# YuxiaWu/RAG4DyG

Measured on AMD Instinct MI355X. Metric: query-seqs/sec encode+top-k over full pool, higher is better.
Workload: dtype f32 (f16x2 operands: two fp16 terms, three products, f32 accumulate)

## Files before the change

### include/r4d.h

```cpp
#ifndef R4D_H
#define R4D_H

#include <stddef.h>
#include <stdint.h>

#ifdef __cplusplus
extern "C" {
#endif

#define R4D_OK 0
#define R4D_ERR_INVALID (-1)
#define R4D_ERR_HIP (-2)
#define R4D_ERR_WORKSPACE (-3)

#define R4D_ABI_VERSION 6

int r4d_abi_version(void);
int r4d_build_flags(void);
const char* r4d_last_error(void);

typedef struct r4d_gpt2_config {
    int32_t n_layer;
    int32_t n_head;
    int32_t n_embd;
// ... 13 lines not shown
    const float* c_fc_wT;     const float* mlp_proj_wT;
    const uint16_t* c_attn_w3;  const uint16_t* attn_proj_w3;
    const uint16_t* c_fc_w3;    const uint16_t* mlp_proj_w3;
    const uint16_t* c_attn_w3t; const uint16_t* attn_proj_w3t;
    const uint16_t* c_fc_w3t;   const uint16_t* mlp_proj_w3t;
    const float* c_attn_wTg;    const float* c_attn_lnc;
    const float* c_fc_wTg;      const float* c_fc_lnc;
    const uint16_t* c_attn_h2;  const uint16_t* attn_proj_h2;
    const uint16_t* c_fc_h2;    const uint16_t* mlp_proj_h2;
} r4d_gpt2_layer;

typedef struct r4d_gpt2_weights {
    const float* wte;
    const float* wpe;
    const float* ln_f_w;
    const float* ln_f_b;
    const r4d_gpt2_layer* layers;
    const float* lm_head;
} r4d_gpt2_weights;


size_t r4d_gpt2_workspace_bytes(const r4d_gpt2_config* cfg, int32_t B, int32_t T);

int r4d_gpt2_encode_f32(const r4d_gpt2_config* cfg, const r4d_gpt2_weights* w,
                        const int64_t* ids_d, const float* inputs_embeds_d, int32_t B, int32_t T,
                        float* out_hidden_d, float* out_meanpool_d, float* out_layers_d, float* out_qkv_d,
                        void* workspace_d, size_t workspace_bytes, void* stream);

size_t r4d_gpt2_groups_workspace_bytes(const r4d_gpt2_config* cfg, int32_t n_groups, const int32_t* Bs,
                                       const int32_t* Ts);
int r4d_gpt2_encode_groups_f32(const r4d_gpt2_config* cfg, const r4d_gpt2_weights* w, int32_t n_groups,
                               const int64_t* const* ids_d, const int32_t* Bs, const int32_t* Ts,
                               float* out_meanpool_d, void* workspace_d, size_t workspace_bytes, void* stream);

int r4d_gpt2_encode_groups_ex_f32(const r4d_gpt2_config* cfg, const r4d_gpt2_weights* w, int32_t n_groups,
                                  const int64_t* const* ids_d, const float* const* embeds_d, const int32_t* Bs,
                                  const int32_t* Ts, float* out_hidden_d, float* out_meanpool_d, float* out_qkv_d,
                                  void* workspace_d, size_t workspace_bytes, void* stream);

size_t r4d_gpt2_decode_workspace_bytes(const r4d_gpt2_config* cfg, int32_t B);
int r4d_gpt2_decode_step_f32(const r4d_gpt2_config* cfg, const r4d_gpt2_weights* w, const int64_t* ids_d,
                             const float* inputs_embeds_d, const int32_t* pos_d, float* kv_cache_d, int32_t B,
                             int32_t t_cap, float* out_hidden_d, void* workspace_d, size_t workspace_bytes,
                             void* stream);

typedef struct r4d_greedy_state {
    float* last_d;
    float* logits_d;
    int64_t* next_d;
    int32_t* lens_d;
    int32_t* pos_d;
    int32_t* active_d;
    int32_t* gen_len_d;
    int32_t* out_tokens_d;
    const int32_t* params_d;
    int32_t out_cap;
} r4d_greedy_state;
typedef struct r4d_decode_graph r4d_decode_graph;

size_t r4d_gpt2_greedy_workspace_bytes(const r4d_gpt2_config* cfg, int32_t B);
int r4d_gpt2_greedy_step_f32(const r4d_gpt2_config* cfg, const r4d_gpt2_weights* w, const r4d_greedy_state* st,
                             float* kv_cache_d, int32_t B, int32_t t_cap, void* workspace_d, size_t workspace_bytes,
                             void* stream);
int r4d_gpt2_greedy_graph_create(const r4d_gpt2_config* cfg, const r4d_gpt2_weights* w, const r4d_greedy_state* st,
                                 float* kv_cache_d, int32_t B, int32_t t_cap, void* workspace_d, size_t workspace_bytes,
                                 r4d_decode_graph** out_graph);
// ... 211 lines not shown
```

### rag4dyg_amd/_lib.py

```python
import ctypes
import os
from ctypes import POINTER, Structure, c_char_p, c_double, c_float, c_int32, c_int64, c_size_t, c_uint32, c_uint64, c_void_p

PKG = os.path.dirname(os.path.abspath(__file__))
LIB_PATH = os.environ.get("R4D_LIB_PATH") or os.path.join(PKG, "librag4dyg_hip.so")

R4D_ABI_VERSION = 6
HEAD_GRAD_UNTIED, HEAD_GRAD_TIED, HEAD_GRAD_NONE = 0, 1, 2


class R4DError(RuntimeError):
    pass


class GPT2ConfigC(Structure):
    _fields_ = [("n_layer", c_int32), ("n_head", c_int32), ("n_embd", c_int32), ("vocab", c_int32),
                ("n_positions", c_int32), ("ln_eps", c_float)]


class GPT2LayerC(Structure):
    _fields_ = [(n, c_void_p) for n in ("ln_1_w", "ln_1_b", "c_attn_w", "c_attn_b", "attn_proj_w", "attn_proj_b",
                                         "ln_2_w", "ln_2_b", "c_fc_w", "c_fc_b", "mlp_proj_w", "mlp_proj_b",
                                         "c_attn_wT", "attn_proj_wT", "c_fc_wT", "mlp_proj_wT",
                                         "c_attn_w3", "attn_proj_w3", "c_fc_w3", "mlp_proj_w3",
                                         "c_attn_w3t", "attn_proj_w3t", "c_fc_w3t", "mlp_proj_w3t",
                                         "c_attn_wTg", "c_attn_lnc", "c_fc_wTg", "c_fc_lnc",
                                         "c_attn_h2", "attn_proj_h2", "c_fc_h2", "mlp_proj_h2")]


class GreedyStateC(Structure):
    _fields_ = [(n, c_void_p) for n in ("last_d", "logits_d", "next_d", "lens_d", "pos_d", "active_d", "gen_len_d",
                                         "out_tokens_d", "params_d")] + [("out_cap", c_int32)]


class GPT2LayerGradsC(Structure):
    _fields_ = [(n, c_void_p) for n in ("ln_1_w", "ln_1_b", "c_attn_w", "c_attn_b", "attn_proj_w", "attn_proj_b",
                                         "ln_2_w", "ln_2_b", "c_fc_w", "c_fc_b", "mlp_proj_w", "mlp_proj_b")]


class TrainDropoutC(Structure):
    _fields_ = [("embd_p", c_float), ("attn_p", c_float), ("resid_p", c_float), ("seed", c_uint64), ("step", c_uint64)]


class GPT2GradsC(Structure):
    _fields_ = [("wte", c_void_p), ("wpe", c_void_p), ("ln_f_w", c_void_p), ("ln_f_b", c_void_p),
                ("layers", POINTER(GPT2LayerGradsC))]


class LMHeadC(Structure):
    _fields_ = [("wte_pad", c_void_p), ("ldV", c_int32), ("w3", c_void_p), ("w3t", c_void_p), ("h2", c_void_p)]


class GPT2WeightsC(Structure):
    _fields_ = [("wte", c_void_p), ("wpe", c_void_p), ("ln_f_w", c_void_p), ("ln_f_b", c_void_p),
                ("layers", POINTER(GPT2LayerC)), ("lm_head", c_void_p)]


_P = c_void_p
PROTOTYPES = {
    "r4d_abi_version": (c_int32, []),
    "r4d_build_flags": (c_int32, []),
    "r4d_last_error": (c_char_p, []),
    "r4d_gpt2_workspace_bytes": (c_size_t, [POINTER(GPT2ConfigC), c_int32, c_int32]),
    "r4d_gpt2_encode_f32": (c_int32, [POINTER(GPT2ConfigC), POINTER(GPT2WeightsC), _P, _P, c_int32, c_int32,
                                      _P, _P, _P, _P, _P, c_size_t, _P]),
    "r4d_gpt2_groups_workspace_bytes": (c_size_t, [POINTER(GPT2ConfigC), c_int32, POINTER(c_int32), POINTER(c_int32)]),
    "r4d_gpt2_encode_groups_f32": (c_int32, [POINTER(GPT2ConfigC), POINTER(GPT2WeightsC), c_int32, POINTER(_P),
                                             POINTER(c_int32), POINTER(c_int32), _P, _P, c_size_t, _P]),
    "r4d_gpt2_encode_groups_ex_f32": (c_int32, [POINTER(GPT2ConfigC), POINTER(GPT2WeightsC), c_int32, POINTER(_P), POINTER(_P),
                                                POINTER(c_int32), POINTER(c_int32), _P, _P, _P, _P, c_size_t, _P]),
    "r4d_set_attention_fused": (c_int32, [c_int32]),
    "r4d_set_attention_h2": (c_int32, [c_int32]),
    "r4d_set_attention_kblk": (c_int32, [c_int32]),
    "r4d_set_layer0_pad_rows": (c_int32, [c_int32]),
    "r4d_gpt2_layer0_pad_rows_offset": (c_size_t, [POINTER(GPT2ConfigC), c_int32, POINTER(c_int32), POINTER(c_int32)]),
    "r4d_pack_kblk_words": (c_int32, [_P, c_int64, c_int32, c_int32, _P, _P]),
    "r4d_attention_h2_kblk_f32": (c_int32, [_P, _P, c_int32, c_int32, c_int32, c_int32, _P, _P]),
    "r4d_set_range_flag": (c_int32, [_P]),
    "r4d_set_gemm_h2p": (c_int32, [c_int32]),
    "r4d_layernorm_lines_f32": (c_int32, [_P, _P, _P, c_int32, c_int32, c_float, _P, _P]),
    "r4d_split2_lines_f16": (c_int32, [_P, c_int64, c_int32, _P, _P]),
    "r4d_conv1d_h2p_f32": (c_int32, [_P, _P, _P, _P, c_int32, c_int32, c_int32, c_int32, c_int32, _P, _P]),
    "r4d_pack_h2_words_f32": (c_int32, [_P, c_int64, _P, _P]),
    "r4d_attention_h2_f32": (c_int32, [_P, c_int32, c_int32, c_int32, c_int32, _P, _P]),
    "r4d_gpt2_decode_workspace_bytes": (c_size_t, [POINTER(GPT2ConfigC), c_int32]),
    "r4d_gpt2_decode_step_f32": (c_int32, [POINTER(GPT2ConfigC), POINTER(GPT2WeightsC), _P, _P, _P, _P, c_int32, c_int32,
                                           _P, _P, c_size_t, _P]),
    "r4d_gpt2_greedy_workspace_bytes": (c_size_t, [POINTER(GPT2ConfigC), c_int32]),
    "r4d_gpt2_greedy_step_f32": (c_int32, [POINTER(GPT2ConfigC), POINTER(GPT2WeightsC), POINTER(GreedyStateC), _P, c_int32,
                                           c_int32, _P, c_size_t, _P]),
    "r4d_gpt2_greedy_graph_create": (c_int32, [POINTER(GPT2ConfigC), POINTER(GPT2WeightsC), POINTER(GreedyStateC), _P,
                                               c_int32, c_int32, _P, c_size_t, POINTER(_P)]),
    "r4d_decode_graph_launch": (c_int32, [_P, c_int32, _P]),
    "r4d_decode_graph_destroy": (None, [_P]),
    "r4d_lm_logits_f32": (c_int32, [_P, _P, c_int32, c_int32, c_int32, _P, _P]),
    "r4d_layernorm_f32": (c_int32, [_P, _P, _P, c_int32, c_int32, c_float, _P, _P]),
    "r4d_conv1d_f32": (c_int32, [_P, _P, _P, _P, _P, c_int32, c_int32, c_int32, c_int32, _P, _P]),
    "r4d_split3_planes_bf16": (c_int32, [_P, c_int32, c_int32, c_int32, _P, _P]),
    "r4d_conv1d_s3_f32": (c_int32, [_P, _P, _P, _P, c_int32, c_int32, c_int32, c_int32, _P, _P]),
    "r4d_split2_planes_f16": (c_int32, [_P, c_int32, c_int32, c_int32, _P, _P]),
    "r4d_conv1d_h2_f32": (c_int32, [_P, _P, _P, _P, c_int32, c_int32, c_int32, c_int32, _P, _P]),
    "r4d_fold_layernorm_f32": (c_int32, [_P, _P, _P, c_int32, c_int32, _P, _P, _P]),
    "r4d_set_gemm_split3": (c_int32, [c_int32]),
# ... 115 lines not shown
```

### rag4dyg_amd/csrc/common.h

```cpp
#pragma once
#include <hip/hip_runtime.h>
#include <stdint.h>
#include <stdio.h>
#include <stdarg.h>
#include "../../include/r4d.h"
#include "conv1d_route.h"

namespace r4d {

void set_error(const char* fmt, ...);
int dbgflag_kc(); int dbgflag_att(); int dbgflag_sk(); int dbgflag_jac(); int dbgflag_scan(); int dbgflag_s3(); int dbgflag_h2();

#define R4D_REQUIRE(cond, ...)                     \
    do {                                           \
        if (!(cond)) {                             \
            r4d::set_error(__VA_ARGS__);           \
            return R4D_ERR_INVALID;                \
        }                                          \
    } while (0)

#define R4D_HIP(call)                                                                  \
    do {                                                                               \
        hipError_t e_ = (call);                                                        \
        if (e_ != hipSuccess) {                                                        \
// ... 22 lines not shown
void prof_begin_impl(int cls, double work, hipStream_t s);
void prof_end_impl(hipStream_t s);
struct ProfScope {
    hipStream_t s; bool on;
    ProfScope(int cls, double work, hipStream_t st) : s(st), on(g_prof_on) { if (on) prof_begin_impl(cls, work, s); }
    ~ProfScope() { if (on) prof_end_impl(s); }
};

#define R4D_BRANCH_LIST(X)                                                                                              \
    X(KC_128x128x16, "gemm_kc:128x128x16") X(KC_128x64x16, "gemm_kc:128x64x16") X(KC_64x64x32, "gemm_kc:64x64x32")       \
    X(KC_128x128x32, "tuning:gemm_kc:128x128x32") X(KC_ROWSPLIT, "gemm_kc:row-split (two launches)")                      \
    X(S3_128x256, "gemm_s3:128x256x32") X(S3_PERSISTENT, "gemm_s3:128x256x32 persistent (pipeline across tiles)") X(S3_128x128, "gemm_s3:128x128x32") X(S3_F32B, "gemm_s3:both operands split on the fly (scoring GEMM)") X(S3_TN, "gemm_s3tn:128x256x32 (weight gradients, transposing LDS reads)")      \
    X(H2_128x256, "gemm_h2:128x256x32 (f16x2)") X(H2_128x128, "gemm_h2:128x128x32 (f16x2)") X(H2P_128x256, "gemm_h2p:128x256x32 (f16x2, A as lines, LDS-DMA)") X(H2P_128x128, "gemm_h2p:128x128x32 (f16x2, A as lines, LDS-DMA)") X(H2P_ROWMAP, "gemm_h2p:row-block map (layer 0 c_attn without the repeated pad-row blocks)") \
    X(F32_128x128, "gemm_f32:128x128") X(F32_128x64, "gemm_f32:128x64") X(F32_64x64, "gemm_f32:64x64")                   \
    X(F32_NT, "gemm_f32:B as [N,K]") X(F32_NN, "gemm_f32:B as [K,N]") X(TN_SPLITK, "gemm_tn:split-K") X(TN_SINGLE, "gemm_tn:one slice") \
    X(SK16_NG2, "skinny16:ng2") X(SK16_NG3, "skinny16:ng3") X(SK16_NG2_LN, "skinny16:ng2+layernorm") X(SK16_LN_FOLDED, "skinny16:LayerNorm pre-folded into the weight") X(SK16_NG3_LN, "skinny16:ng3+layernorm") \
    X(SK16_SPLITK, "skinny16:split-K last-arriver") X(SK8_NG2, "skinny8:ng2") X(SK8_NG3, "skinny8:ng3")                    \
    X(SK8_LN, "tuning:skinny8:+layernorm") X(SK8_SPLITK, "skinny8:split-K + epilogue launch") X(SK_PLAIN, "skinny:plain + epilogue launch") \
    X(ATT_KS32, "attention:key-split hd32") X(ATT_KS64, "attention:key-split hd64") X(ATT_CS96, "attention:column-split hd96") \
    X(ATT_CS128, "attention:column-split hd128") X(ATT_CS256, "attention:column-split hd256") X(ATT_H2_KS32, "attention:f16x2 key-split hd32") X(ATT_H2_KS64, "attention:f16x2 key-split hd64") X(ATT_H2_KS96, "attention:f16x2 key-split hd96") X(ATT_H2_128, "attention:f16x2 hd128") X(ATT_H2_256, "attention:f16x2 hd256") X(ATT_H2_KS32_KBLK, "attention:f16x2 key-split hd32, key-blocked K") X(ATT_H2_KS64_KBLK, "attention:f16x2 key-split hd64, key-blocked K") X(ATT_H2_KS96_KBLK, "attention:f16x2 key-split hd96, key-blocked K") X(ATT_H2_128_KBLK, "attention:f16x2 hd128, key-blocked K") X(ATT_H2_256_KBLK, "attention:f16x2 hd256, key-blocked K")                              \
    X(ATT_KS_FORCED, "tuning:attention:key-split at hd96/128/256") X(ATT_3LAUNCH, "attention:three-launch GEMM form")      \
    X(SCAN_1_1, "scan:d32") X(SCAN_2_1, "scan:d64") X(SCAN_4_1, "scan:d128") X(SCAN_4_2, "scan:d256") X(SCAN_4_3, "scan:d384") \
    X(SCAN_8_2, "scan:d512") X(SCAN_4_4, "tuning:scan:d512 4-way") X(SCAN_8_3, "scan:d768") X(SCAN_8_4, "scan:d1024")       \
    X(SCAN_SHORT, "scan:short shard (even rows, two tiles in flight)") X(SCAN_DMA, "scan:short shard, LDS-DMA staged") X(SCAN_RING, "scan:long shard, LDS-DMA ring") X(SCAN_GEMM, "scan:tiled GEMM (Q > 64 or other d)") X(SCAN_TILED, "scan:128x256 tiles in the scan kernels' arithmetic (Q >= 64)") X(SCAN_BF16X3, "scan:bf16x3 operands") X(SCAN_F32, "scan:exact-f32 operands")  \
    X(TOPK_ONE_WG, "topk:one workgroup per row") X(TOPK_TICKET, "topk:cross-workgroup ticket merge")                      \
    X(TOPK_MULTI, "topk:second launch over candidates") X(TOPK_F64, "topk:f64 rows")                                      \
    X(EMBED_LN4, "embed+layernorm:16-byte lanes") X(EMBED_GENERIC, "embed+layernorm:generic") X(LN4_2, "layernorm:ln4<2>") X(LN4_4, "layernorm:ln4<4>") X(LN4_8, "layernorm:ln4<8>") X(LN_GENERIC, "layernorm:generic") \
    X(LNF_8, "lnf_meanpool:<8>") X(LNF_16, "lnf_meanpool:<16>") X(LNF_32, "lnf_meanpool:<32>")                             \
    X(DEC_ATT_32, "decode_attention:<32>") X(DEC_ATT_64, "decode_attention:<64>")                                         \
    X(JAC_LDS, "jaccard:LDS table") X(JAC_MERGE, "jaccard:merge walk (vocab too large for LDS)")                          \
    X(JAC_PREP_DENSE_LDS, "jaccard_prep:dense tokens, LDS histogram") X(JAC_PREP_DENSE_GLOBAL, "jaccard_prep:dense tokens, global histogram") X(JAC_PREP_ORDER, "jaccard_prep:rows longest first") \
    X(ARGSORT_ONE, "argsort:one chunk") X(ARGSORT_MULTI, "argsort:chunk sort + rank scatter")                              \
    X(B1_128x256, "tuning:encode_bf16:128x256x32") X(B1_128x128, "tuning:encode_bf16:128x128x32")                           \
    X(TB_FWD, "tuning:train_bf16:fwd") X(TB_DGRAD, "tuning:train_bf16:dgrad") X(TB_WGRAD, "tuning:train_bf16:wgrad") X(TB_WGRAD_FALLBACK, "tuning:train_bf16:wgrad_fallback")
enum DispatchBranch {
#define X(id, name) BR_##id,
    R4D_BRANCH_LIST(X)
#undef X
    BR_COUNT
};
extern unsigned long long g_branch_hits[BR_COUNT];
#define R4D_BRANCH(id) (++r4d::g_branch_hits[r4d::BR_##id])

extern unsigned* g_range_flag;

static inline size_t align_up(size_t x, size_t a) { return (x + a - 1) / a * a; }

enum GemmCausal { CAUSAL_NONE = 0, CAUSAL_QK = 1, CAUSAL_PV = 2 };

struct GemmArgs {
    const float* A; const float* B; float* C;
    const float* bias;
    const float* resid;
    int M, N, K;
    int lda, ldb, ldc, ldr;
    int b_trans;
    int b_rows;
    int a_cols;
    int nbatch, nb1;
    long long sA0, sA1, sB0, sB1, sC0, sC1;
    int epilogue; float scale_div;
    int causal;
};
static inline GemmArgs gemm_args(const float* A, const float* B, int b_trans, const float* bias, const float* resid, int M, int K, int N,
                                 int epilogue, float* C) {
    GemmArgs g{};
    g.A = A; g.B = B; g.C = C; g.bias = bias; g.resid = resid;
// ... 184 lines not shown
```

### rag4dyg_amd/csrc/encoder.hip

```cpp
#include <math.h>
#include <stdlib.h>
#include <string.h>
#include <vector>
#include "common.h"

namespace r4d {

static thread_local char g_err[512] = "";
void set_error(const char* fmt, ...) {
    va_list ap;
    va_start(ap, fmt);
    vsnprintf(g_err, sizeof(g_err), fmt, ap);
    va_end(ap);
}

int g_gemm_split3 = 1;
int g_encode_bf16 = 0;

int conv1d(const Conv1DW& W, const float* x, const float* resid, int M, int epilogue, float* y, hipStream_t s, const Conv1DOpts& opts) {
    const int K = W.in, N = W.out;
    const GemmRoute route = conv1d_route(W, M, epilogue, opts.skinny_scratch != nullptr, opts.bf16);
    switch (route) {
        case ROUTE_B1:
            if (opts.bf16 == BF16_TRAIN) R4D_BRANCH(TB_FWD);
            return launch_gemm_b1(s3_args(x, W.w3, W.b, resid, M, K, N, epilogue, y), s);
        case ROUTE_SKINNY:
            return launch_gemm_skinny(x, W.wT, W.b, resid, M, K, N, epilogue, y, opts.skinny_scratch, s, nullptr, nullptr, 0.f,
                                      opts.counters_zeroed);
        case ROUTE_H2: return launch_gemm_h2(s3_args(x, W.h2, W.b, resid, M, K, N, epilogue, y), s);
        case ROUTE_S3: return launch_gemm_s3(s3_args(x, W.w3, W.b, resid, M, K, N, epilogue, y), s);
        default: break;
    }
    R4D_REQUIRE(epilogue != EPI_H2WORDS, "conv1d: the h2-word epilogue exists in the f16x2 GEMM only");
    const bool kcopy = route == ROUTE_F32_KCOPY;
    return launch_gemm_f32(gemm_args(x, kcopy ? W.wT : W.w, kcopy, W.b, resid, M, K, N, epilogue, y), s);
// ... 65 lines not shown
    size_t pad_rows_off;
    size_t bytes;
};
static Workspace carve(void* base, size_t M, size_t score_floats, size_t pool_floats, int d, const PadRowsPlan* pr = nullptr) {
    size_t off = 0;
    auto take = [&](size_t nfloat) {
        float* p = base ? (float*)((char*)base + off) : nullptr;
        off += align_up(nfloat * sizeof(float), 256);
        return p;
    };
    const size_t Mx = pr ? pr->rows() : M;
    Workspace w;
    w.x = take(Mx * d); w.ln = take(Mx * d); w.qkv = take(Mx * 3 * d); w.att = take(M * d); w.fc = take(M * 4 * d);
    w.scores = take(score_floats);
    w.pool = take(pool_floats);
    w.kblk = reinterpret_cast<unsigned*>(take(kblk_words(Mx, d)));
    w.pad_rows_off = off;
    w.pad_rows = pr ? reinterpret_cast<int*>(take(pr->words())) : nullptr;
    w.bytes = off;
    return w;
}
static int g_layer0_pad_rows = -1;
static int layer0_pad_rows_on() {
    if (g_layer0_pad_rows < 0) { const char* e = getenv("R4D_LAYER0_PAD_ROWS"); g_layer0_pad_rows = e ? atoi(e) != 0 : 1; }
    return g_layer0_pad_rows;
}
static PadRowsPlan groups_pad_rows_plan(const r4d_gpt2_config* cfg, size_t M, int n_groups, const int32_t* Ts) {
    int Tmax = 1;
    for (int g = 0; g < n_groups; ++g) Tmax = Ts[g] > Tmax ? Ts[g] : Tmax;
    return pad_rows_plan(M, Tmax, cfg->vocab > 0 ? cfg->vocab : 1);
}
static size_t score_floats(int B, int H, int T) { return (size_t)B * H * T * tpad(T); }

static int check_cfg(const r4d_gpt2_config* c) {
    R4D_REQUIRE(c != nullptr, "gpt2: null config");
    R4D_REQUIRE(c->n_layer >= 1 && c->n_head >= 1 && c->n_embd >= 64, "gpt2: bad config L=%d H=%d d=%d", c->n_layer,
                c->n_head, c->n_embd);
    R4D_REQUIRE(c->n_embd % 64 == 0 && c->n_embd <= 2048, "gpt2: n_embd=%d must be a multiple of 64, <= 2048", c->n_embd);
    R4D_REQUIRE(c->n_embd % c->n_head == 0 && (c->n_embd / c->n_head) % 16 == 0,
                "gpt2: head_dim=%d/%d must be a multiple of 16", c->n_embd, c->n_head);
    return R4D_OK;
}

}

using namespace r4d;

extern "C" {

int r4d_abi_version(void) { return R4D_ABI_VERSION; }
int r4d_build_flags(void) {
    return dbgflag_kc() | (dbgflag_att() << 1) | (dbgflag_sk() << 2) | (dbgflag_jac() << 3) | (dbgflag_scan() << 4) | (dbgflag_s3() << 5) | (dbgflag_h2() << 6) | (dbgflag_att_h2() << 7);
}
int r4d_fold_layernorm_f32(const float* wT_d, const float* ln_w_d, const float* ln_b_d, int32_t N, int32_t K, float* wTg_d,
                           float* lnc_d, void* stream) {
    return launch_fold_layernorm(wT_d, ln_w_d, ln_b_d, N, K, wTg_d, lnc_d, (hipStream_t)stream);
}

int r4d_set_gemm_split3(int32_t mode) { g_gemm_split3 = mode == 2 ? 2 : (mode != 0); return R4D_OK; }
int r4d_get_gemm_split3(void) { return g_gemm_split3; }
int r4d_set_encode_bf16(int32_t on) {
    const int prev = g_encode_bf16;
    g_encode_bf16 = on != 0;
    return prev;
}
int r4d_get_encode_bf16(void) { return g_encode_bf16; }
int r4d_set_range_flag(uint32_t* flag_d) { g_range_flag = flag_d; return R4D_OK; }
int r4d_set_attention_kblk(int32_t on) {
    const int prev = g_attention_kblk < 0 ? 1 : g_attention_kblk;
    g_attention_kblk = on != 0;
    return prev;
}
int r4d_set_attention_h2(int32_t on) {
    const int prev = g_attention_h2;
    g_attention_h2 = on != 0;
    return prev;
}

int r4d_set_attention_fused(int32_t mode) {
    g_attention_variant = (mode == 2) ? 1 : 0;
    g_attention_fused = mode < 0 ? -1 : (mode != 0);
    return R4D_OK;
}
const char* r4d_last_error(void) { return g_err; }

size_t r4d_gpt2_workspace_bytes(const r4d_gpt2_config* cfg, int32_t B, int32_t T) {
    if (!cfg || B <= 0 || T <= 0) return 0;
    const PadRowsPlan pr = groups_pad_rows_plan(cfg, (size_t)B * T, 1, &T);
    return carve(nullptr, (size_t)B * T, score_floats(B, cfg->n_head, T), lnf_meanpool_scratch_floats(B, T, cfg->n_embd),
                 cfg->n_embd, &pr).bytes;
}

size_t r4d_gpt2_groups_workspace_bytes(const r4d_gpt2_config* cfg, int32_t n_groups, const int32_t* Bs,
                                       const int32_t* Ts) {
    if (!cfg || n_groups <= 0 || !Bs || !Ts) return 0;
    size_t M = 0, sc = 0, pl = 0;
    for (int g = 0; g < n_groups; ++g) {
        if (Bs[g] <= 0 || Ts[g] <= 0) return 0;
        M += (size_t)Bs[g] * Ts[g];
        const size_t f = score_floats(Bs[g], cfg->n_head, Ts[g]);
        if (f > sc) sc = f;
        pl += lnf_meanpool_scratch_floats(Bs[g], Ts[g], cfg->n_embd);
    }
    const PadRowsPlan pr = groups_pad_rows_plan(cfg, M, n_groups, Ts);
    return carve(nullptr, M, sc, pl, cfg->n_embd, &pr).bytes;
}

size_t r4d_gpt2_layer0_pad_rows_offset(const r4d_gpt2_config* cfg, int32_t n_groups, const int32_t* Bs, const int32_t* Ts) {
    if (!cfg || n_groups <= 0 || !Bs || !Ts) return 0;
    size_t M = 0, sc = 0, pl = 0;
    for (int g = 0; g < n_groups; ++g) {
        if (Bs[g] <= 0 || Ts[g] <= 0) return 0;
        M += (size_t)Bs[g] * Ts[g];
        const size_t f = score_floats(Bs[g], cfg->n_head, Ts[g]);
        if (f > sc) sc = f;
        pl += lnf_meanpool_scratch_floats(Bs[g], Ts[g], cfg->n_embd);
    }
    const PadRowsPlan pr = groups_pad_rows_plan(cfg, M, n_groups, Ts);
    return carve(nullptr, M, sc, pl, cfg->n_embd, &pr).pad_rows_off;
}

int r4d_set_layer0_pad_rows(int32_t on) {
    const int prev = layer0_pad_rows_on();
    g_layer0_pad_rows = on != 0;
    return prev;
}

}

namespace r4d {

static int encode_impl(const r4d_gpt2_config* cfg, const r4d_gpt2_weights* w, const Group* groups, int n_groups,
                       float* out_hidden_d, float* out_meanpool_d, float* out_layers_d, float* out_qkv_d,
                       void* workspace_d, size_t workspace_bytes, hipStream_t s) {
    int rc = check_cfg(cfg);
    if (rc) return rc;
    R4D_REQUIRE(w && w->wte && w->wpe && w->ln_f_w && w->ln_f_b && w->layers, "gpt2: null weights");
    R4D_REQUIRE(out_hidden_d || out_meanpool_d, "gpt2: no output requested");
    const int d = cfg->n_embd, H = cfg->n_head;
    size_t Mtot = 0, sc = 0, pl = 0;
    int Tmax = 1;
    bool all_ids = true;
    for (int g = 0; g < n_groups; ++g) {
        const Group& G = groups[g];
        Tmax = G.T > Tmax ? G.T : Tmax;
        all_ids = all_ids && G.ids != nullptr;
        R4D_REQUIRE((G.ids != nullptr) != (G.emb != nullptr),
                    "gpt2: specify exactly one of input_ids and inputs_embeds");
        R4D_REQUIRE(G.B >= 1 && G.T >= 1, "gpt2: empty batch B=%d T=%d", G.B, G.T);
        R4D_REQUIRE(G.T <= cfg->n_positions && G.T <= 1024, "gpt2: T=%d exceeds n_positions=%d", G.T, cfg->n_positions);
        Mtot += (size_t)G.B * G.T;
        const size_t f = score_floats(G.B, H, G.T);
        if (f > sc) sc = f;
// ... 104 lines not shown
        }
        if (!fused_done) {
            for (int g = 0; g < n_groups; ++g) {
                const Group& G = groups[g];
                if ((rc = attention(qkv + G.row0 * 3 * d, G.B, G.T, H, d, ws.att + G.row0 * d, ws.scores, s))) return rc;
            }
        }
        if (att_lines) rc = conv1d_lines(Wo, reinterpret_cast<const unsigned short*>(ws.att), ws.x, M, EPI_RESIDUAL, ws.x, false, s);
        else rc = conv1d(Wo, ws.att, ws.x, M, EPI_RESIDUAL, ws.x, s, enc);
        if (rc) return rc;
        if (lines) {
            if ((rc = launch_layernorm_lines(ws.x, L.ln_2_w, L.ln_2_b, M, d, cfg->ln_eps, ln_lines, s))) return rc;
            if ((rc = conv1d_lines(Wfc, ln_lines, nullptr, M, EPI_GELU, fc_lines, true, s))) return rc;
            if ((rc = conv1d_lines(Wp, fc_lines, ws.x, M, EPI_RESIDUAL, ws.x, false, s))) return rc;
            continue;
        }
        if ((rc = launch_layernorm(ws.x, L.ln_2_w, L.ln_2_b, M, d, cfg->ln_eps, ws.ln, s))) return rc;
        if ((rc = conv1d(Wfc, ws.ln, nullptr, M, EPI_GELU, ws.fc, s, enc))) return rc;
        if ((rc = conv1d(Wp, ws.fc, ws.x, M, EPI_RESIDUAL, ws.x, s, enc))) return rc;
    }
    size_t part0 = 0;
    for (int g0 = 0; g0 < n_groups; g0 += ATT_MAXG) {
        const RowGroups R = row_groups(groups, g0, n_groups);
        const Group& G = groups[g0];
        rc = launch_lnf_meanpool_groups(R, ws.x + G.row0 * d, w->ln_f_w, w->ln_f_b, d, cfg->ln_eps,
                                        out_hidden_d ? out_hidden_d + G.row0 * d : nullptr,
                                        out_meanpool_d ? out_meanpool_d + G.seq0 * d : nullptr, ws.pool + part0, s);
        if (rc) return rc;
        for (int j = 0; j < R.n; ++j) part0 += lnf_meanpool_scratch_floats(R.B[j], R.T[j], d);
    }
    return R4D_OK;
}

}

extern "C" {

int r4d_gpt2_encode_f32(const r4d_gpt2_config* cfg, const r4d_gpt2_weights* w, const int64_t* ids_d,
                        const float* inputs_embeds_d, int32_t B, int32_t T, float* out_hidden_d,
                        float* out_meanpool_d, float* out_layers_d, float* out_qkv_d, void* workspace_d,
                        size_t workspace_bytes, void* stream) {
    Group G = {ids_d, inputs_embeds_d, B, T, 0, 0};
    return encode_impl(cfg, w, &G, 1, out_hidden_d, out_meanpool_d, out_layers_d, out_qkv_d, workspace_d,
                       workspace_bytes, (hipStream_t)stream);
}

int r4d_gpt2_encode_groups_f32(const r4d_gpt2_config* cfg, const r4d_gpt2_weights* w, int32_t n_groups,
                               const int64_t* const* ids_d, const int32_t* Bs, const int32_t* Ts,
                               float* out_meanpool_d, void* workspace_d, size_t workspace_bytes, void* stream) {
    R4D_REQUIRE(n_groups >= 1 && n_groups <= 4096 && ids_d && Bs && Ts, "gpt2 groups: bad arguments");
    R4D_REQUIRE(out_meanpool_d, "gpt2 groups: out_meanpool_d is null");
    std::vector<Group> gs((size_t)n_groups);
    size_t row0 = 0, seq0 = 0;
    for (int g = 0; g < n_groups; ++g) {
        gs[g] = Group{ids_d[g], nullptr, Bs[g], Ts[g], row0, seq0};
        if (Bs[g] > 0 && Ts[g] > 0) { row0 += (size_t)Bs[g] * Ts[g]; seq0 += (size_t)Bs[g]; }
    }
    return encode_impl(cfg, w, gs.data(), n_groups, nullptr, out_meanpool_d, nullptr, nullptr, workspace_d,
                       workspace_bytes, (hipStream_t)stream);
}

int r4d_gpt2_encode_groups_ex_f32(const r4d_gpt2_config* cfg, const r4d_gpt2_weights* w, int32_t n_groups,
                                  const int64_t* const* ids_d, const float* const* embeds_d, const int32_t* Bs,
                                  const int32_t* Ts, float* out_hidden_d, float* out_meanpool_d, float* out_qkv_d,
                                  void* workspace_d, size_t workspace_bytes, void* stream) {
    R4D_REQUIRE(n_groups >= 1 && n_groups <= 4096 && Bs && Ts, "gpt2 groups: bad arguments");
    R4D_REQUIRE((ids_d != nullptr) != (embeds_d != nullptr), "gpt2 groups: specify exactly one of ids_d and embeds_d");
    std::vector<Group> gs((size_t)n_groups);
    size_t row0 = 0, seq0 = 0;
    for (int g = 0; g < n_groups; ++g) {
        gs[g] = Group{ids_d ? ids_d[g] : nullptr, embeds_d ? embeds_d[g] : nullptr, Bs[g], Ts[g], row0, seq0};
        if (Bs[g] > 0 && Ts[g] > 0) { row0 += (size_t)Bs[g] * Ts[g]; seq0 += (size_t)Bs[g]; }
    }
    return encode_impl(cfg, w, gs.data(), n_groups, out_hidden_d, out_meanpool_d, nullptr, out_qkv_d, workspace_d,
                       workspace_bytes, (hipStream_t)stream);
}

static size_t decode_skinny_floats(int d) {
    size_t m = 0;
    const int shapes[4][2] = {{d, 3 * d}, {d, d}, {d, 4 * d}, {4 * d, d}};
    for (auto& kn : shapes)
        if (gemm_skinny_supported(1, kn[0], kn[1])) { const size_t f = gemm_skinny_scratch_floats(kn[0], kn[1]); if (f > m) m = f; }
    return m;
}

size_t r4d_gpt2_decode_workspace_bytes(const r4d_gpt2_config* cfg, int32_t B) {
    if (!cfg || B <= 0) return 0;
    return carve(nullptr, (size_t)B, 0, decode_skinny_floats(cfg->n_embd), cfg->n_embd).bytes;
}

static int skinny_ln(const Conv1DW& W, const float* x, const float* ln_w, const float* ln_b, float eps, int M, int epilogue, float* y,
                     float* sk, hipStream_t s) {
// ... 215 lines not shown
```

### rag4dyg_amd/ops.py

```python
import torch

from . import _lib
from ._lib import check


def _stream():
    return torch.cuda.current_stream().cuda_stream


def _dev(t, dtype, name):
    if not isinstance(t, torch.Tensor) or not t.is_cuda:
        raise _lib.R4DError(f"{name}: expected a tensor on the GPU (no CPU fallback in rag4dyg_amd)")
    if t.dtype != dtype:
        raise _lib.R4DError(f"{name}: expected dtype {dtype}, got {t.dtype}")
    if not t.is_contiguous():
        raise _lib.R4DError(f"{name}: tensor must be contiguous")
    return t.data_ptr()


_WS = {}


def workspace(nbytes, device, tag="default"):
    key = (str(device), tag)
    buf = _WS.get(key)
    if buf is None or buf.numel() < nbytes:
        buf = torch.empty(max(int(nbytes), 256), dtype=torch.uint8, device=device)
        _WS[key] = buf
    return buf


def layernorm(x, w, b, eps=1e-5):
# ... 231 lines not shown
        if not t.is_cuda or t.dtype != torch.float32 or t.dim() != 2 or t.stride(1) != 1:
            raise R4DError(f"weight_grad_bf16: {n} must be a 2-D fp32 device tensor with contiguous rows")
    rows, n_in = x.shape
    n_out = dy.shape[1]
    if dy.shape[0] != rows:
        raise R4DError("weight_grad_bf16: x and dy differ in rows")
    nbytes = lib.r4d_weight_grad_bf16_workspace_bytes(rows, n_in, n_out)
    if workspace is None:
        workspace = torch.empty(max(int(nbytes), 256), dtype=torch.uint8, device=x.device)
    dw = torch.empty(n_in, n_out, dtype=torch.float32, device=x.device)
    db = torch.empty(n_out, dtype=torch.float32, device=x.device) if want_db else None
    check(lib.r4d_weight_grad_bf16_f32(x.data_ptr(), int(x.stride(0)), dy.data_ptr(), int(dy.stride(0)), rows, n_in, n_out, dw.data_ptr(),
                                       db.data_ptr() if want_db else None, workspace.data_ptr(), workspace.numel(), _stream()),
          "weight_grad_bf16")
    return dw, db


def set_attention_fused(mode):
    _lib.load().r4d_set_attention_fused(-1 if mode is None or mode == -1 else (2 if mode == 2 else int(bool(mode))))


def set_attention_h2(on):
    return bool(_lib.load().r4d_set_attention_h2(int(bool(on))))


def set_attention_kblk(on):
    return bool(_lib.load().r4d_set_attention_kblk(int(bool(on))))


def set_layer0_pad_rows(on):
    return bool(_lib.load().r4d_set_layer0_pad_rows(int(bool(on))))


def pack_kblk_words(qkv_words, n_head):
    B, T, d3 = qkv_words.shape
    d = d3 // 3
    rows = B * T
    out = torch.empty((rows + 31) // 32 * 32 * d, dtype=torch.int32, device=qkv_words.device)
    check(_lib.load().r4d_pack_kblk_words(_dev(qkv_words, torch.int32, "qkv_words"), rows, n_head, d, out.data_ptr(), _stream()), "pack_kblk_words")
    return out


def attention_h2_kblk(qkv_words, kblk, n_head):
    B, T, d3 = qkv_words.shape
    d = d3 // 3
    a = torch.empty(B, T, d, dtype=torch.float32, device=qkv_words.device)
    check(_lib.load().r4d_attention_h2_kblk_f32(_dev(qkv_words, torch.int32, "qkv_words"), _dev(kblk, torch.int32, "kblk"), B, T, n_head, d,
                                                a.data_ptr(), _stream()), "attention_h2_kblk")
    return a


def pack_h2_words(x):
    x = x.contiguous()
    w = torch.empty(x.shape, dtype=torch.int32, device=x.device)
    check(_lib.load().r4d_pack_h2_words_f32(_dev(x, torch.float32, "x"), x.numel(), w.data_ptr(), _stream()), "pack_h2_words")
    return w


def attention_h2(qkv_words, n_head):
    B, T, d3 = qkv_words.shape
    d = d3 // 3
    a = torch.empty(B, T, d, dtype=torch.float32, device=qkv_words.device)
    check(_lib.load().r4d_attention_h2_f32(_dev(qkv_words, torch.int32, "qkv_words"), B, T, n_head, d, a.data_ptr(), _stream()),
          "attention_h2")
    return a

# ... 162 lines not shown
```

Measured before the change: 41630.

## Split grouped encode across two HIP streams to overlap independent group halves

Splits the grouped GPT-2 encode into two row-balanced halves at a group boundary and runs the second half on an internal non-blocking stream, joined back with events. Each half gets its own carved workspace region, so the workspace size query now returns the larger two-part layout. The aim is to fill the GPU when a single encode_impl launch chain leaves compute units idle, at the cost of more workspace and per-call event/stream overhead. The split is skipped under profiling, graph capture, or when the smaller half is below a fill heuristic.

```diff
diff --git a/include/r4d.h b/include/r4d.h
--- a/include/r4d.h
+++ b/include/r4d.h
@@ -69,6 +69,18 @@
 int r4d_gpt2_encode_groups_f32(const r4d_gpt2_config* cfg, const r4d_gpt2_weights* w, int32_t n_groups,
                                const int64_t* const* ids_d, const int32_t* Bs, const int32_t* Ts,
                                float* out_meanpool_d, void* workspace_d, size_t workspace_bytes, void* stream);
+
+typedef struct r4d_encode_split {
+    int32_t split;
+    int32_t n_first;
+    uint64_t rows[2];
+    uint64_t offset[2];
+    uint64_t bytes[2];
+} r4d_encode_split;
+int r4d_encode_split_plan(const r4d_gpt2_config* cfg, int32_t n_groups, const int32_t* Bs, const int32_t* Ts, r4d_encode_split* plan);
+int r4d_set_encode_split_min_rows(int32_t min_rows);
+int r4d_set_encode_streams(int32_t n);
+int r4d_get_encode_streams(void);
 
 int r4d_gpt2_encode_groups_ex_f32(const r4d_gpt2_config* cfg, const r4d_gpt2_weights* w, int32_t n_groups,
                                   const int64_t* const* ids_d, const float* const* embeds_d, const int32_t* Bs,
diff --git a/rag4dyg_amd/_lib.py b/rag4dyg_amd/_lib.py
--- a/rag4dyg_amd/_lib.py
+++ b/rag4dyg_amd/_lib.py
@@ -26,6 +26,10 @@
                                          "c_attn_w3t", "attn_proj_w3t", "c_fc_w3t", "mlp_proj_w3t",
                                          "c_attn_wTg", "c_attn_lnc", "c_fc_wTg", "c_fc_lnc",
                                          "c_attn_h2", "attn_proj_h2", "c_fc_h2", "mlp_proj_h2")]
+
+
+class EncodeSplitC(Structure):
+    _fields_ = [("split", c_int32), ("n_first", c_int32), ("rows", c_uint64 * 2), ("offset", c_uint64 * 2), ("bytes", c_uint64 * 2)]
 
 
 class GreedyStateC(Structure):
@@ -69,6 +73,10 @@
                                              POINTER(c_int32), POINTER(c_int32), _P, _P, c_size_t, _P]),
     "r4d_gpt2_encode_groups_ex_f32": (c_int32, [POINTER(GPT2ConfigC), POINTER(GPT2WeightsC), c_int32, POINTER(_P), POINTER(_P),
                                                 POINTER(c_int32), POINTER(c_int32), _P, _P, _P, _P, c_size_t, _P]),
+    "r4d_encode_split_plan": (c_int32, [POINTER(GPT2ConfigC), c_int32, POINTER(c_int32), POINTER(c_int32), POINTER(EncodeSplitC)]),
+    "r4d_set_encode_split_min_rows": (c_int32, [c_int32]),
+    "r4d_set_encode_streams": (c_int32, [c_int32]),
+    "r4d_get_encode_streams": (c_int32, []),
     "r4d_set_attention_fused": (c_int32, [c_int32]),
     "r4d_set_attention_h2": (c_int32, [c_int32]),
     "r4d_set_attention_kblk": (c_int32, [c_int32]),
diff --git a/rag4dyg_amd/csrc/common.h b/rag4dyg_amd/csrc/common.h
--- a/rag4dyg_amd/csrc/common.h
+++ b/rag4dyg_amd/csrc/common.h
@@ -78,7 +78,8 @@
     X(JAC_PREP_DENSE_LDS, "jaccard_prep:dense tokens, LDS histogram") X(JAC_PREP_DENSE_GLOBAL, "jaccard_prep:dense tokens, global histogram") X(JAC_PREP_ORDER, "jaccard_prep:rows longest first") \
     X(ARGSORT_ONE, "argsort:one chunk") X(ARGSORT_MULTI, "argsort:chunk sort + rank scatter")                              \
     X(B1_128x256, "tuning:encode_bf16:128x256x32") X(B1_128x128, "tuning:encode_bf16:128x128x32")                           \
-    X(TB_FWD, "tuning:train_bf16:fwd") X(TB_DGRAD, "tuning:train_bf16:dgrad") X(TB_WGRAD, "tuning:train_bf16:wgrad") X(TB_WGRAD_FALLBACK, "tuning:train_bf16:wgrad_fallback")
+    X(TB_FWD, "tuning:train_bf16:fwd") X(TB_DGRAD, "tuning:train_bf16:dgrad") X(TB_WGRAD, "tuning:train_bf16:wgrad") X(TB_WGRAD_FALLBACK, "tuning:train_bf16:wgrad_fallback") \
+    X(ENC_TWO_STREAMS, "tuning:encode:two streams")
 enum DispatchBranch {
 #define X(id, name) BR_##id,
     R4D_BRANCH_LIST(X)
diff --git a/rag4dyg_amd/csrc/encoder.hip b/rag4dyg_amd/csrc/encoder.hip
--- a/rag4dyg_amd/csrc/encoder.hip
+++ b/rag4dyg_amd/csrc/encoder.hip
@@ -1,6 +1,7 @@
 #include <math.h>
 #include <stdlib.h>
 #include <string.h>
+#include <mutex>
 #include <vector>
 #include "common.h"
 
@@ -132,6 +133,57 @@
 }
 static size_t score_floats(int B, int H, int T) { return (size_t)B * H * T * tpad(T); }
 
+static Workspace groups_layout(const r4d_gpt2_config* cfg, int n_groups, const int32_t* Bs, const int32_t* Ts) {
+    Workspace none = {};
+    if (!cfg || n_groups <= 0 || !Bs || !Ts) return none;
+    size_t M = 0, sc = 0, pl = 0;
+    for (int g = 0; g < n_groups; ++g) {
+        if (Bs[g] <= 0 || Ts[g] <= 0) return none;
+        M += (size_t)Bs[g] * Ts[g];
+        const size_t f = score_floats(Bs[g], cfg->n_head, Ts[g]);
+        if (f > sc) sc = f;
+        pl += lnf_meanpool_scratch_floats(Bs[g], Ts[g], cfg->n_embd);
+    }
+    const PadRowsPlan pr = groups_pad_rows_plan(cfg, M, n_groups, Ts);
+    return carve(nullptr, M, sc, pl, cfg->n_embd, &pr);
+}
+
+static int g_encode_streams = -1;
+static int g_encode_split_min_rows = 0;
+static int encode_streams() {
+    if (g_encode_streams < 0) { const char* e = getenv("R4D_ENCODE_STREAMS"); g_encode_streams = (e && atoi(e) == 1) ? 1 : 2; }
+    return g_encode_streams;
+}
+static int encode_split_plan(const r4d_gpt2_config* cfg, int n_groups, const int32_t* Bs, const int32_t* Ts, r4d_encode_split* plan) {
+    R4D_REQUIRE(cfg && plan && n_groups >= 1 && Bs && Ts && cfg->n_embd >= 1, "encode_split_plan: bad arguments");
+    size_t M = 0;
+    for (int g = 0; g < n_groups; ++g) {
+        R4D_REQUIRE(Bs[g] >= 1 && Ts[g] >= 1, "encode_split_plan: empty batch B=%d T=%d", Bs[g], Ts[g]);
+        M += (size_t)Bs[g] * Ts[g];
+    }
+    memset(plan, 0, sizeof(*plan));
+    plan->n_first = n_groups; plan->rows[0] = M;
+    size_t first = 0, best_first = 0, best_gap = M + 1;
+    int cut = 0;
+    for (int g = 0; g + 1 < n_groups; ++g) {
+        first += (size_t)Bs[g] * Ts[g];
+        const size_t second = M - first, gap = first > second ? first - second : second - first;
+        if (gap < best_gap) { best_gap = gap; best_first = first; cut = g + 1; }
+    }
+    const size_t smaller = best_first < M - best_first ? best_first : M - best_first;
+    const bool fills = g_encode_split_min_rows > 0 ? smaller >= (size_t)g_encode_split_min_rows
+                                                   : (smaller + 127) / 128 * (((size_t)cfg->n_embd + 255) / 256) >= 256;
+    if (cut > 0 && fills) {
+        plan->split = 1; plan->n_first = cut; plan->rows[0] = best_first; plan->rows[1] = M - best_first;
+    }
+    plan->bytes[0] = groups_layout(cfg, plan->n_first, Bs, Ts).bytes;
+    if (plan->split) {
+        plan->offset[1] = plan->bytes[0];
+        plan->bytes[1] = groups_layout(cfg, n_groups - cut, Bs + cut, Ts + cut).bytes;
+    }
+    return R4D_OK;
+}
+
 static int check_cfg(const r4d_gpt2_config* c) {
     R4D_REQUIRE(c != nullptr, "gpt2: null config");
     R4D_REQUIRE(c->n_layer >= 1 && c->n_head >= 1 && c->n_embd >= 64, "gpt2: bad config L=%d H=%d d=%d", c->n_layer,
@@ -193,32 +245,31 @@
 
 size_t r4d_gpt2_groups_workspace_bytes(const r4d_gpt2_config* cfg, int32_t n_groups, const int32_t* Bs,
                                        const int32_t* Ts) {
-    if (!cfg || n_groups <= 0 || !Bs || !Ts) return 0;
-    size_t M = 0, sc = 0, pl = 0;
-    for (int g = 0; g < n_groups; ++g) {
-        if (Bs[g] <= 0 || Ts[g] <= 0) return 0;
-        M += (size_t)Bs[g] * Ts[g];
-        const size_t f = score_floats(Bs[g], cfg->n_head, Ts[g]);
-        if (f > sc) sc = f;
-        pl += lnf_meanpool_scratch_floats(Bs[g], Ts[g], cfg->n_embd);
-    }
-    const PadRowsPlan pr = groups_pad_rows_plan(cfg, M, n_groups, Ts);
-    return carve(nullptr, M, sc, pl, cfg->n_embd, &pr).bytes;
+    const size_t one = groups_layout(cfg, n_groups, Bs, Ts).bytes;
+    r4d_encode_split sp;
+    if (!one || encode_split_plan(cfg, n_groups, Bs, Ts, &sp) || !sp.split) return one;
+    const size_t two = (size_t)(sp.offset[1] + sp.bytes[1]);
+    return two > one ? two : one;
 }
 
 size_t r4d_gpt2_layer0_pad_rows_offset(const r4d_gpt2_config* cfg, int32_t n_groups, const int32_t* Bs, const int32_t* Ts) {
-    if (!cfg || n_groups <= 0 || !Bs || !Ts) return 0;
-    size_t M = 0, sc = 0, pl = 0;
-    for (int g = 0; g < n_groups; ++g) {
-        if (Bs[g] <= 0 || Ts[g] <= 0) return 0;
-        M += (size_t)Bs[g] * Ts[g];
-        const size_t f = score_floats(Bs[g], cfg->n_head, Ts[g]);
-        if (f > sc) sc = f;
-        pl += lnf_meanpool_scratch_floats(Bs[g], Ts[g], cfg->n_embd);
-    }
-    const PadRowsPlan pr = groups_pad_rows_plan(cfg, M, n_groups, Ts);
-    return carve(nullptr, M, sc, pl, cfg->n_embd, &pr).pad_rows_off;
-}
+    return groups_layout(cfg, n_groups, Bs, Ts).pad_rows_off;
+}
+
+int r4d_encode_split_plan(const r4d_gpt2_config* cfg, int32_t n_groups, const int32_t* Bs, const int32_t* Ts, r4d_encode_split* plan) {
+    return encode_split_plan(cfg, n_groups, Bs, Ts, plan);
+}
+int r4d_set_encode_split_min_rows(int32_t min_rows) {
+    const int prev = g_encode_split_min_rows;
+    g_encode_split_min_rows = min_rows > 0 ? min_rows : 0;
+    return prev;
+}
+int r4d_set_encode_streams(int32_t n) {
+    const int prev = encode_streams();
+    g_encode_streams = n >= 2 ? 2 : 1;
+    return prev;
+}
+int r4d_get_encode_streams(void) { return encode_streams(); }
 
 int r4d_set_layer0_pad_rows(int32_t on) {
     const int prev = layer0_pad_rows_on();
@@ -389,6 +440,29 @@
     return R4D_OK;
 }
 
+struct EncodeFork { hipStream_t stream; hipEvent_t fork, join; bool ready; };
+static std::mutex g_fork_mu;
+static EncodeFork* encode_fork() {
+    static EncodeFork forks[64] = {};
+    int devi = 0;
+    if (hipGetDevice(&devi) != hipSuccess || devi < 0 || devi >= 64) { set_error("gpt2: no current device for the internal stream"); return nullptr; }
+    EncodeFork& f = forks[devi];
+    if (f.ready) return &f;
+    if (hipStreamCreateWithFlags(&f.stream, hipStreamNonBlocking) != hipSuccess) { set_error("gpt2: creating the internal stream failed"); return nullptr; }
+    if (hipEventCreateWithFlags(&f.fork, hipEventDisableTiming) != hipSuccess) {
+        (void)hipStreamDestroy(f.stream);
+        set_error("gpt2: creating the fork event failed");
+        return nullptr;
+    }
+    if (hipEventCreateWithFlags(&f.join, hipEventDisableTiming) != hipSuccess) {
+        (void)hipEventDestroy(f.fork); (void)hipStreamDestroy(f.stream);
+        set_error("gpt2: creating the join event failed");
+        return nullptr;
+    }
+    f.ready = true;
+    return &f;
+}
+
 }
 
 extern "C" {
@@ -413,8 +487,39 @@
         gs[g] = Group{ids_d[g], nullptr, Bs[g], Ts[g], row0, seq0};
         if (Bs[g] > 0 && Ts[g] > 0) { row0 += (size_t)Bs[g] * Ts[g]; seq0 += (size_t)Bs[g]; }
     }
-    return encode_impl(cfg, w, gs.data(), n_groups, nullptr, out_meanpool_d, nullptr, nullptr, workspace_d,
-                       workspace_bytes, (hipStream_t)stream);
+    hipStream_t s = (hipStream_t)stream;
+    r4d_encode_split sp;
+    bool two = encode_streams() == 2 && !g_prof_on && cfg && n_groups >= 2;
+    for (int g = 0; g < n_groups && two; ++g) two = Bs[g] >= 1 && Ts[g] >= 1;
+    if (two) two = encode_split_plan(cfg, n_groups, Bs, Ts, &sp) == R4D_OK && sp.split;
+    if (two) {
+        hipStreamCaptureStatus cst = hipStreamCaptureStatusNone;
+        if (hipStreamIsCapturing(s, &cst) != hipSuccess) { (void)hipGetLastError(); two = false; }
+        else two = cst == hipStreamCaptureStatusNone;
+    }
+    if (!two)
+        return encode_impl(cfg, w, gs.data(), n_groups, nullptr, out_meanpool_d, nullptr, nullptr, workspace_d, workspace_bytes, s);
+    if (!workspace_d || workspace_bytes < sp.offset[1] + sp.bytes[1]) {
+        set_error("gpt2: workspace %zu bytes < required %zu", workspace_bytes, (size_t)(sp.offset[1] + sp.bytes[1]));
+        return R4D_ERR_WORKSPACE;
+    }
+    const size_t rows0 = gs[sp.n_first].row0;
+    for (int g = sp.n_first; g < n_groups; ++g) gs[g].row0 -= rows0;
+    std::lock_guard<std::mutex> lock(g_fork_mu);
+    EncodeFork* f = encode_fork();
+    if (!f) return R4D_ERR_HIP;
+    R4D_HIP(hipEventRecord(f->fork, s));
+    R4D_HIP(hipStreamWaitEvent(f->stream, f->fork, 0));
+    R4D_BRANCH(ENC_TWO_STREAMS);
+    int rc = encode_impl(cfg, w, gs.data(), sp.n_first, nullptr, out_meanpool_d, nullptr, nullptr, (char*)workspace_d + sp.offset[0],
+                         (size_t)sp.bytes[0], s);
+    if (rc == R4D_OK)
+        rc = encode_impl(cfg, w, gs.data() + sp.n_first, n_groups - sp.n_first, nullptr, out_meanpool_d, nullptr, nullptr,
+                         (char*)workspace_d + sp.offset[1], (size_t)sp.bytes[1], f->stream);
+    if (hipEventRecord(f->join, f->stream) != hipSuccess || hipStreamWaitEvent(s, f->join, 0) != hipSuccess) {
+        if (rc == R4D_OK) { set_error("gpt2: joining the internal stream failed"); rc = R4D_ERR_HIP; }
+    }
+    return rc;
 }
 
 int r4d_gpt2_encode_groups_ex_f32(const r4d_gpt2_config* cfg, const r4d_gpt2_weights* w, int32_t n_groups,
diff --git a/rag4dyg_amd/ops.py b/rag4dyg_amd/ops.py
--- a/rag4dyg_amd/ops.py
+++ b/rag4dyg_amd/ops.py
@@ -1,3 +1,5 @@
+import ctypes
+
 import torch
 
 from . import _lib
@@ -295,6 +297,22 @@
     return bool(_lib.load().r4d_set_layer0_pad_rows(int(bool(on))))
 
 
+def set_encode_streams(n):
+    return int(_lib.load().r4d_set_encode_streams(int(n)))
+
+
+def set_encode_split_min_rows(rows):
+    return int(_lib.load().r4d_set_encode_split_min_rows(int(rows or 0)))
+
+
+def encode_split_plan(cfg, Bs, Ts):
+    n = len(Bs)
+    sp = _lib.EncodeSplitC()
+    check(_lib.load().r4d_encode_split_plan(ctypes.byref(cfg), n, (ctypes.c_int32 * n)(*Bs), (ctypes.c_int32 * n)(*Ts), ctypes.byref(sp)),
+          "encode_split_plan")
+    return dict(split=bool(sp.split), n_first=int(sp.n_first), rows=tuple(sp.rows), offset=tuple(sp.offset), bytes=tuple(sp.bytes))
+
+
 def pack_kblk_words(qkv_words, n_head):
     B, T, d3 = qkv_words.shape
     d = d3 // 3
```

Result: no change. 41970, median of 6 (+0.8%).
